# Andurdur/Chroma-Subsampling-Image-Compressor

Measured on AMD Instinct MI355X. Metric: Mpixels/s end-to-end (RGB->YCbCr->4:2:0->reconstruct), higher is better.
Workload: dtype u8

## Files before the change

chroma-subsampling-image-compressor_amd/csrc/csic_pack.hip:

```cpp
#include <cstdio>

#include "csic_pack_common.h"

namespace csic {

template <int Q, bool NT>
__global__ void __launch_bounds__(PK_T) k_pack_widths(PkArgs e)
{
    __shared__ uint32_t s_w[PK_T], s_a[PK_T], s_tot[PK_WAVES];
    const int plane = e.plane0 + (int)blockIdx.y;
    const uint32_t G = e.groups[plane], g0 = blockIdx.x * PK_T, t = threadIdx.x;
    if (g0 >= G) return;
    const gpdst_t cb = pk_coded_frame(e);
    uint32_t w = 0, anchor = 0;
    if (g0 + t < G) {
        uint32_t u[32];
        w = pk_fold_group<Q, NT>(e, pk_bits_frame(e), plane, g0 + t, u, anchor);
    }
    s_w[t] = w;
    s_a[t] = anchor;
    uint32_t total;
    (void)pk_block_scan(w, s_tot, total);
    if (t == 0) *pk_ws(e, blockIdx.z, e.block0[plane] + blockIdx.x) = total;
    pk_store_sections<Q>(e, cb, plane, G, g0, s_w, s_a);
}

__global__ void __launch_bounds__(PK_T) k_pack_scan(PkArgs e)
{
    __shared__ uint32_t s_tot[PK_WAVES];
    uint32_t carry = 0;
    for (uint32_t b0 = 0; b0 < e.nblocks; b0 += PK_T) {
        const uint32_t b = b0 + threadIdx.x;
        const uint32_t v = b < e.nblocks ? *pk_ws(e, blockIdx.x, b) : 0u;
        uint32_t total;
        const uint32_t before = pk_block_scan(v, s_tot, total);
        if (b < e.nblocks) *pk_ws(e, blockIdx.x, b) = carry + before;
        carry += total;
    }
    if (threadIdx.x == 0 && e.sizes)
        ((unsigned long long CSIC_GLOBAL *)(uintptr_t)e.sizes)[blockIdx.x] = (unsigned long long)e.payload_offset + 4ull * carry;
}

template <int Q, bool NT>
__global__ void __launch_bounds__(PK_T) k_pack_emit(PkArgs e)
{
    __shared__ uint32_t s_tot[PK_WAVES];
    const int plane = e.plane0 + (int)blockIdx.y;
    const uint32_t G = e.groups[plane], g0 = blockIdx.x * PK_T, t = threadIdx.x;
    if (g0 >= G) return;
    uint32_t u[32], w = 0, anchor = 0;
#pragma unroll
    for (int j = 0; j < 32; ++j) u[j] = 0;
    if (g0 + t < G) w = pk_fold_group<Q, NT>(e, pk_bits_frame(e), plane, g0 + t, u, anchor);
    uint32_t total;
    const uint32_t before = pk_block_scan(w, s_tot, total);
    if (w == 0) return;
    const gpdst_t cb = pk_coded_frame(e);
    int64_t at = e.payload_offset + 4 * ((int64_t)*pk_ws(e, blockIdx.z, e.block0[plane] + blockIdx.x) + before);
    uint64_t acc = 0;
    uint32_t fill = 0;
#pragma unroll
    for (int j = 0; j < 32; ++j) {
        acc |= (uint64_t)u[j] << fill;
        fill += w;
        if (fill >= 32u) {
            pk_coded_st4(e, cb, at, (uint32_t)acc);
            at += 4;
            acc >>= 32;
            fill -= 32u;
        }
    }
}

__device__ __forceinline__ uint32_t pk_width(const PkArgs &e, gpdst_t cb, int plane, uint32_t g)
{
    return min(pk_nibble(e, cb, plane, g), (uint32_t)e.q[plane]);
}

__global__ void __launch_bounds__(PK_T) k_unpack_sums(PkArgs e)
{
    __shared__ uint32_t s_tot[PK_WAVES];
    const int plane = (int)blockIdx.y;
    const uint32_t G = e.groups[plane], g0 = blockIdx.x * PK_T, t = threadIdx.x;
    if (g0 >= G) return;
    const uint32_t w = g0 + t < G ? pk_width(e, pk_coded_frame(e), plane, g0 + t) : 0u;
    uint32_t total;
    (void)pk_block_scan(w, s_tot, total);
    if (t == 0) *pk_ws(e, blockIdx.z, e.block0[plane] + blockIdx.x) = total;
}

template <int Q, bool NT>
__global__ void __launch_bounds__(PK_T) k_unpack_emit(PkArgs e)
{
    constexpr uint32_t MASK = (1u << Q) - 1u;
    __shared__ uint32_t s_tot[PK_WAVES];
    const int plane = e.plane0 + (int)blockIdx.y;
    const uint32_t G = e.groups[plane], g0 = blockIdx.x * PK_T, t = threadIdx.x, g = g0 + t;
    if (g0 >= G) return;
    const gpdst_t cb = pk_coded_frame(e);
    const uint32_t w = g < G ? pk_width(e, cb, plane, g) : 0u;
    uint32_t total;
    const uint32_t before = pk_block_scan(w, s_tot, total);
    if (g >= G) return;
    uint32_t c = pk_anchor<Q>(e, cb, plane, g);
    const uint32_t n = e.n[plane], wmask = (1u << w) - 1u;
    int64_t at = e.payload_offset + 4 * ((int64_t)*pk_ws(e, blockIdx.z, e.block0[plane] + blockIdx.x) + before);
    uint64_t acc = 0;
    uint32_t have = 0;
    PkGroupOut<Q> out;
#pragma unroll
    for (int j = 0; j < 32; ++j) {
        if (have < w) {
            acc |= (uint64_t)pk_coded_ld4(e, cb, at) << have;
            at += 4;
            have += 32u;
        }
        const uint32_t uu = (uint32_t)acc & wmask;
        acc >>= w;
        have -= w;
        if (j > 0) c = (c + rice_unfold(uu, MASK)) & MASK;
        out.put(j, 32u * g + (uint32_t)j < n ? c : 0u);
    }
    out.template store<NT>(e, pk_bits_frame(e), plane, g);
}

int pk_fill_args(const csic_plan *pl, const PackGeometry &G, const int64_t (&nibbles_offset)[3], const int64_t (&anchors_offset)[3],
                 int64_t payload_offset, int64_t bound_bytes, const char *entry, PkArgs *e)
{
    *e = PkArgs{};
    if ((int64_t)pl->g.W * pl->g.H >= ((int64_t)1 << 31)) return set_error(CSIC_EINVAL_SIZE, "frame too large for %s", entry);
    e->frame_bytes = G.bits.frame_bytes;
    e->bound_bytes = bound_bytes;
    e->payload_offset = payload_offset;
    for (int p = 0; p < 3; ++p) {
        e->off[p] = G.src_offset[p];
        e->bytes[p] = G.src_bytes[p];
        e->n[p] = (uint32_t)G.n[p];
        e->groups[p] = (uint32_t)G.layout.groups[p];
        e->q[p] = G.q[p];
        e->woff[p] = (uint32_t)nibbles_offset[p];
        e->aoff[p] = (uint32_t)anchors_offset[p];
        e->adw[p] = (uint32_t)((G.layout.groups[p] * G.q[p] + 31) / 32);
        e->block0[p] = (uint32_t)G.block0[p];
    }
    e->nblocks = (uint32_t)G.nblocks;
    return CSIC_OK;
}

static int fill_pk_args(const csic_plan *pl, PkArgs *e)
{
    PackGeometry G;
    const int st = pack_geometry(&pl->p, &G);
    if (st != CSIC_OK) return st;
    return pk_fill_args(pl, G, G.layout.widths_offset, G.layout.anchors_offset, G.layout.payload_offset, G.layout.bound_bytes, "csic_pack_device", e);
}

static const auto pack_widths = [](auto q, auto nt) { return k_pack_widths<CSIC_CONST(q), CSIC_CONST(nt)>; };
static const auto pack_emit = [](auto q, auto nt) { return k_pack_emit<CSIC_CONST(q), CSIC_CONST(nt)>; };
static const auto unpack_emit = [](auto q, auto nt) { return k_unpack_emit<CSIC_CONST(q), CSIC_CONST(nt)>; };

static int pk_launch(void (*fn)(PkArgs), PkArgs &e, dim3 grid, hipStream_t stream)
{
    void *params[1] = {&e};
    HIP_TRY(hipLaunchKernel(reinterpret_cast<const void *>(fn), grid, dim3(PK_T, 1, 1), params, 0, stream));
    return CSIC_OK;
}

int pack_scan_launch(PkArgs &e, int nframes, hipStream_t stream) { return pk_launch(k_pack_scan, e, dim3((unsigned)nframes, 1, 1), stream); }

int pk_check_buffers(const csic_plan *plan, const void *d_bits, const void *d_coded, int32_t nframes, bool has_ws, const void *d_workspace)
{
    if (!plan) return set_error(CSIC_EINVAL_NULL, "plan is NULL");
    if (!d_bits || !d_coded || (has_ws && !d_workspace)) return set_error(CSIC_EINVAL_NULL, "device buffer is NULL");
    if (nframes < 1 || nframes > 65535) return set_error(CSIC_EINVAL_SIZE, "nframes must be 1..65535. Got %d", nframes);
    if (((uintptr_t)d_bits | (uintptr_t)d_coded) & 255u) return set_error(CSIC_EINVAL_SIZE, "PLANAR_BITS and coded frame buffers must be 256-byte aligned");
    if (has_ws && ((uintptr_t)d_workspace & 7u)) return set_error(CSIC_EINVAL_SIZE, "d_workspace must be 8-byte aligned");
    return CSIC_OK;
}

const char *pk_kernel_name(const char *family, const csic_plan *plan)
{
    static thread_local char buf[64];
    if (!plan) return "";
    std::snprintf(buf, sizeof buf, "%s<q%d,%d,%d,%s>", family, plan->p.y_bits, plan->p.cb_bits, plan->p.cr_bits, plan->tune.no_nt ? "cached" : "nt");
    return buf;
}

}

using namespace csic;

extern "C" {

const char *csic_pack_kernel_name(const csic_plan *plan) { return pk_kernel_name("k_pack", plan); }

int csic_pack_workspace_bytes(const csic_plan *plan, int32_t nframes, size_t *bytes) { return pk_workspace_bytes(plan, nframes, bytes, fill_pk_args); }

int csic_pack_device(csic_plan *plan, const void *d_bits, int32_t nframes, void *d_coded, uint64_t *d_sizes, void *d_workspace,
                     size_t workspace_bytes, void *hip_stream)
{
    if (plan && !d_sizes) return set_error(CSIC_EINVAL_NULL, "d_sizes is NULL");
    PkArgs e;
    int st = pk_prepare(plan, d_bits, d_coded, nframes, true, d_workspace, workspace_bytes, fill_pk_args, &e);
    if (st != CSIC_OK) return st;
    if ((uintptr_t)d_sizes & 7u) return set_error(CSIC_EINVAL_SIZE, "d_sizes must be 8-byte aligned");
    e.sizes = reinterpret_cast<unsigned long long *>(d_sizes);
    hipStream_t stream = static_cast<hipStream_t>(hip_stream);
    CSIC_DEVICE_SCOPE(plan->device);
    if ((st = pk_launch_planes(plan, e, nframes, stream, pack_widths)) != CSIC_OK) return st;
    if ((st = pack_scan_launch(e, nframes, stream)) != CSIC_OK) return st;
    if ((st = pk_launch_planes(plan, e, nframes, stream, pack_emit)) != CSIC_OK) return st;
    clear_error();
    return CSIC_OK;
}

int csic_unpack_device(csic_plan *plan, const void *d_coded, int32_t nframes, void *d_bits, void *d_workspace, size_t workspace_bytes,
                       void *hip_stream)
{
    PkArgs e;
    int st = pk_prepare(plan, d_bits, d_coded, nframes, true, d_workspace, workspace_bytes, fill_pk_args, &e);
    if (st != CSIC_OK) return st;
    hipStream_t stream = static_cast<hipStream_t>(hip_stream);
    CSIC_DEVICE_SCOPE(plan->device);
    uint32_t gmax = 0;
    for (int p = 0; p < 3; ++p) gmax = e.groups[p] > gmax ? e.groups[p] : gmax;
    if ((st = pk_launch(k_unpack_sums, e, dim3((gmax + PK_T - 1) / PK_T, 3, (unsigned)nframes), stream)) != CSIC_OK) return st;
    if ((st = pack_scan_launch(e, nframes, stream)) != CSIC_OK) return st;
    if ((st = pk_launch_planes(plan, e, nframes, stream, unpack_emit)) != CSIC_OK) return st;
    clear_error();
    return CSIC_OK;
}

}
```

chroma-subsampling-image-compressor_amd/csrc/csic_pack_common.h:

```cpp
#pragma once
#include "csic_kernel_ops.h"
#include "csic_rice_decode.h"

namespace csic {

typedef const uint8_t CSIC_GLOBAL *gpsrc_t;
typedef uint8_t CSIC_GLOBAL *gpdst_t;

constexpr int PK_T = 256, PK_WAVES = PK_T / 64;
static_assert(PK_T == RICE_BLOCK, "a block of the kernels is a block of the format: pack_geometry numbers both");

struct PkArgs {
    uint8_t *bits;
    uint8_t *coded;
    uint32_t *ws;
    unsigned long long *sizes;
    int64_t frame_bytes, bound_bytes;
    int64_t off[3], bytes[3];
    int64_t payload_offset;
    uint32_t n[3], groups[3];
    int32_t q[3];
    uint32_t woff[3], aoff[3];
    uint32_t adw[3];
    uint32_t block0[3], nblocks;
    int32_t plane0;
};

#if defined(CSIC_DEBUG) && CSIC_DEBUG
#define CSIC_PCHECK(lim, off, cnt) CSIC_CHECK((int64_t)(off) >= 0 && (int64_t)(off) + (cnt) <= (int64_t)(lim))
#else
#define CSIC_PCHECK(lim, off, cnt) do { } while (0)
#endif

template <bool NT> __device__ __forceinline__ uint32_t pk_bits_ld4(const PkArgs &e, gpdst_t fb, int64_t off)
{
    CSIC_PCHECK(e.frame_bytes, off, 4); (void)e;
    return ld1<NT>((gin_t)(fb + off));
}
__device__ __forceinline__ uint32_t pk_bits_ld1(const PkArgs &e, gpdst_t fb, int64_t off)
{
    CSIC_PCHECK(e.frame_bytes, off, 1); (void)e;
    return fb[off];
}
template <bool NT> __device__ __forceinline__ void pk_bits_st4(const PkArgs &e, gpdst_t fb, int64_t off, uint32_t v)
{
    CSIC_PCHECK(e.frame_bytes, off, 4); (void)e;
    st1<NT>((gout_t)(fb + off), v);
}
__device__ __forceinline__ void pk_bits_st1(const PkArgs &e, gpdst_t fb, int64_t off, uint32_t v)
{
    CSIC_PCHECK(e.frame_bytes, off, 1); (void)e;
    fb[off] = (uint8_t)v;
}
__device__ __forceinline__ uint32_t pk_coded_ld4(const PkArgs &e, gpdst_t cb, int64_t off)
{
    CSIC_PCHECK(e.bound_bytes, off, 4); (void)e;
    return *(gin_t)(cb + off);
}
__device__ __forceinline__ void pk_coded_st4(const PkArgs &e, gpdst_t cb, int64_t off, uint32_t v)
{
    CSIC_PCHECK(e.bound_bytes, off, 4); (void)e;
    *(gout_t)(cb + off) = v;
}
__device__ __forceinline__ gout_t pk_ws(const PkArgs &e, uint32_t frame, uint32_t b)
{
    CSIC_CHECK(b < e.nblocks && frame < 65535u);
    return (gout_t)(uintptr_t)e.ws + ((uint64_t)frame * e.nblocks + b);
}

__device__ __forceinline__ gpdst_t pk_bits_frame(const PkArgs &e) { return (gpdst_t)(uintptr_t)e.bits + (int64_t)blockIdx.z * e.frame_bytes; }
__device__ __forceinline__ gpdst_t pk_coded_frame(const PkArgs &e) { return (gpdst_t)(uintptr_t)e.coded + (int64_t)blockIdx.z * e.bound_bytes; }

__device__ __forceinline__ uint32_t pk_block_scan(uint32_t v, uint32_t *s_tot, uint32_t &total)
{
    const uint32_t lane = threadIdx.x & 63u, wave = threadIdx.x >> 6;
    uint32_t inc = v;
#pragma unroll
    for (int d = 1; d < 64; d <<= 1) {
        const uint32_t t = (uint32_t)__shfl_up((int)inc, d, 64);
        if (lane >= (uint32_t)d) inc += t;
    }
    if (lane == 63u) s_tot[wave] = inc;
    __syncthreads();
    uint32_t before = 0;
    total = 0;
#pragma unroll
    for (int k = 0; k < PK_WAVES; ++k) {
        const uint32_t t = s_tot[k];
        if ((uint32_t)k < wave) before += t;
        total += t;
    }
    __syncthreads();
    return before + inc - v;
}

template <int Q, bool NT>
__device__ __forceinline__ uint32_t pk_fold_group(const PkArgs &e, gpdst_t fb, int plane, uint32_t g, uint32_t (&u)[32], uint32_t &anchor)
{
    constexpr uint32_t MASK = (1u << Q) - 1u, HALF = 1u << (Q - 1);
    const uint32_t n = e.n[plane];
    const int64_t base = e.off[plane] + 4 * (int64_t)g * Q;
    const bool whole = 32u * g + 32u <= n;
    uint32_t d[Q];
    if (whole) {
#pragma unroll
        for (int i = 0; i < Q; ++i) d[i] = pk_bits_ld4<NT>(e, fb, base + 4 * i);
    } else {
        const int64_t end = e.off[plane] + e.bytes[plane];
#pragma unroll
        for (int i = 0; i < Q; ++i) {
            d[i] = 0;
#pragma unroll
            for (int k = 0; k < 4; ++k)
                if (base + 4 * i + k < end) d[i] |= pk_bits_ld1(e, fb, base + 4 * i + k) << (8 * k);
        }
    }
    uint32_t c[32];
#pragma unroll
    for (int j = 0; j < 32; ++j) {
        const int w = (j * Q) >> 5, s = (j * Q) & 31;
        uint32_t v = d[w] >> s;
        if (s + Q > 32) v |= d[(w + 1) % Q] << ((32 - s) & 31);
        c[j] = v & MASK;
    }
    if (!whole) {
#pragma unroll
        for (int j = 1; j < 32; ++j)
            if (32u * g + (uint32_t)j >= n) c[j] = c[j - 1];
    }
    anchor = c[0];
    uint32_t any = 0;
    u[0] = 0;
#pragma unroll
    for (int j = 1; j < 32; ++j) {
        const uint32_t r = (c[j] - c[j - 1]) & MASK;
        u[j] = r < HALF ? 2u * r : 2u * (MASK + 1u - r) - 1u;
        any |= u[j];
    }
    return any ? 32u - (uint32_t)__builtin_clz(any) : 0u;
}

template <int Q>
__device__ __forceinline__ void pk_store_sections(const PkArgs &e, gpdst_t cb, int plane, uint32_t G, uint32_t g0, const uint32_t *s_nib, const uint32_t *s_a)
{
    const uint32_t t = threadIdx.x;
    if (t < 32u) {
        if (g0 + 8u * t < G) {
            uint32_t v = 0;
#pragma unroll
            for (int k = 0; k < 8; ++k) v |= s_nib[8u * t + (uint32_t)k] << (4 * k);
            pk_coded_st4(e, cb, (int64_t)e.woff[plane] + 4 * (int64_t)(g0 / 8u + t), v);
        }
    } else if (t >= 64u && t < 64u + 8u * Q) {
        const uint32_t a = t - 64u, dw = blockIdx.x * (8u * Q) + a;
        if (dw < e.adw[plane]) {
            uint32_t v = 0;
            for (uint32_t i = 32u * a / Q; i * Q < 32u * a + 32u; ++i) {
                const int sh = (int)(i * Q) - (int)(32u * a);
                v |= sh >= 0 ? s_a[i] << sh : s_a[i] >> -sh;
            }
            pk_coded_st4(e, cb, (int64_t)e.aoff[plane] + 4 * (int64_t)dw, v);
        }
    }
}

__device__ __forceinline__ uint32_t pk_nibble(const PkArgs &e, gpdst_t cb, int plane, uint32_t g)
{
    return (pk_coded_ld4(e, cb, (int64_t)e.woff[plane] + 4 * (int64_t)(g >> 3)) >> (4u * (g & 7u))) & 15u;
}

template <int Q> __device__ __forceinline__ uint32_t pk_anchor(const PkArgs &e, gpdst_t cb, int plane, uint32_t g)
{
    const uint32_t abit = g * Q, as = abit & 31u;
    const int64_t aat = (int64_t)e.aoff[plane] + 4 * (int64_t)(abit >> 5);
    uint32_t c = pk_coded_ld4(e, cb, aat) >> as;
    if (as + Q > 32u) c |= pk_coded_ld4(e, cb, aat + 4) << (32u - as);
    return c & ((1u << Q) - 1u);
}

template <int Q> struct PkGroupOut {
    uint32_t d[Q];
    __device__ __forceinline__ PkGroupOut()
    {
#pragma unroll
        for (int i = 0; i < Q; ++i) d[i] = 0;
    }
    __device__ __forceinline__ void put(int j, uint32_t v)
    {
        const int wi = (j * Q) >> 5, s = (j * Q) & 31;
        d[wi] |= v << s;
        if (s + Q > 32) d[(wi + 1) % Q] |= v >> ((32 - s) & 31);
    }
    template <bool NT> __device__ __forceinline__ void store(const PkArgs &e, gpdst_t fb, int plane, uint32_t g) const
    {
        const int64_t base = e.off[plane] + 4 * (int64_t)g * Q;
        if (32u * g + 32u <= e.n[plane]) {
#pragma unroll
            for (int i = 0; i < Q; ++i) pk_bits_st4<NT>(e, fb, base + 4 * i, d[i]);
        } else {
            const int64_t end = e.off[plane] + e.bytes[plane];
#pragma unroll
            for (int i = 0; i < Q; ++i)
#pragma unroll
                for (int k = 0; k < 4; ++k)
                    if (base + 4 * i + k < end) pk_bits_st1(e, fb, base + 4 * i + k, (d[i] >> (8 * k)) & 0xFFu);
        }
    }
};

int pk_fill_args(const csic_plan *pl, const PackGeometry &G, const int64_t (&nibbles_offset)[3], const int64_t (&anchors_offset)[3],
                 int64_t payload_offset, int64_t bound_bytes, const char *entry, PkArgs *e);

inline size_t pk_workspace_need(int32_t nframes, uint32_t nblocks) { return ((size_t)nframes * nblocks * sizeof(uint32_t) + 7) / 8 * 8; }

int pk_check_buffers(const csic_plan *plan, const void *d_bits, const void *d_coded, int32_t nframes, bool has_ws, const void *d_workspace);
template <class Args>
int pk_prepare(const csic_plan *plan, const void *d_bits, const void *d_coded, int32_t nframes, bool has_ws, const void *d_workspace,
               size_t workspace_bytes, int (*fill)(const csic_plan *, Args *), Args *e)
{
    int st = pk_check_buffers(plan, d_bits, d_coded, nframes, has_ws, d_workspace);
    if (st == CSIC_OK) st = fill(plan, e);
    if (st != CSIC_OK) return st;
    if (has_ws && workspace_bytes < pk_workspace_need(nframes, e->nblocks))
        return set_error(CSIC_EINVAL_SIZE, "workspace of %zu bytes, %d frames need %zu", workspace_bytes, nframes, pk_workspace_need(nframes, e->nblocks));
    e->bits = const_cast<uint8_t *>(static_cast<const uint8_t *>(d_bits));
    e->coded = const_cast<uint8_t *>(static_cast<const uint8_t *>(d_coded));
    e->ws = const_cast<uint32_t *>(static_cast<const uint32_t *>(d_workspace));
    return CSIC_OK;
}

template <class Args> int pk_workspace_bytes(const csic_plan *plan, int32_t nframes, size_t *bytes, int (*fill)(const csic_plan *, Args *))
{
    if (!plan || !bytes) return set_error(CSIC_EINVAL_NULL, "plan or bytes is NULL");
    if (nframes < 1 || nframes > 65535) return set_error(CSIC_EINVAL_SIZE, "nframes must be 1..65535. Got %d", nframes);
    Args e;
    const int st = fill(plan, &e);
    if (st != CSIC_OK) return st;
    *bytes = pk_workspace_need(nframes, e.nblocks);
    clear_error();
    return CSIC_OK;
}

template <class Args, class Choose> int pk_launch_planes(const csic_plan *plan, Args &e, int nframes, hipStream_t stream, Choose choose)
{
    for (int p0 = 0; p0 < 3;) {
        int p1 = p0 + 1;
        while (p1 < 3 && e.q[p1] == e.q[p0]) ++p1;
        uint32_t gmax = 0;
        for (int p = p0; p < p1; ++p) gmax = e.groups[p] > gmax ? e.groups[p] : gmax;
        if (gmax > 0) {
            e.plane0 = p0;
            void (*const fn)(Args) = with_const<true, false>(!plan->tune.no_nt, [&](auto nt) {
                return with_const<1, 2, 3, 4, 5, 6, 7, 8>(e.q[p0], [&](auto q) -> void (*)(Args) { return choose(q, nt); });
            });
            void *params[1] = {&e};
            HIP_TRY(hipLaunchKernel(reinterpret_cast<const void *>(fn), dim3((gmax + PK_T - 1) / PK_T, (unsigned)(p1 - p0), (unsigned)nframes),
                                    dim3(PK_T, 1, 1), params, 0, stream));
        }
        p0 = p1;
    }
    return CSIC_OK;
}

int pack_scan_launch(PkArgs &e, int nframes, hipStream_t stream);

const char *pk_kernel_name(const char *family, const csic_plan *plan);

}
```

chroma-subsampling-image-compressor_amd/csrc/csic_rice_decode.h:

```cpp
#pragma once
#include <cstdint>

#if defined(__HIPCC__)
#define CSIC_RICE_HD __host__ __device__ inline
#else
#define CSIC_RICE_HD inline
#endif

namespace csic {

CSIC_RICE_HD uint32_t rice_word(const uint32_t *seg, uint32_t nwords, uint32_t i) { return i < nwords ? seg[i] : 0u; }

CSIC_RICE_HD uint32_t rice_bits(const uint32_t *seg, uint32_t nwords, uint32_t bit, uint32_t n)
{
    const uint32_t wi = bit >> 5, sh = bit & 31u;
    uint32_t v = rice_word(seg, nwords, wi) >> sh;
    if (sh + n > 32u) v |= rice_word(seg, nwords, wi + 1u) << (32u - sh);
    return v & ((1u << n) - 1u);
}

CSIC_RICE_HD uint32_t rice_select32(uint32_t w, uint32_t r)
{
    uint32_t pos = 0;
    for (uint32_t s = 16; s >= 1u; s >>= 1) {
        const uint32_t lo = w & ((1u << s) - 1u), c = (uint32_t)__builtin_popcount(lo);
        if (r >= c) { r -= c; w >>= s; pos += s; } else w = lo;
    }
    return (w & 1u) && r == 0 ? pos : 32u;
}

CSIC_RICE_HD uint32_t rice_after_terminator(const uint32_t *words, const uint32_t *cum, uint32_t n, uint32_t t)
{
    if (t == 0) return 0;
    uint32_t lo = 0, hi = n;
    while (lo < hi) {
        const uint32_t mid = lo + ((hi - lo) >> 1);
        if (cum[mid] >= t) hi = mid; else lo = mid + 1u;
    }
    if (lo >= n) return 32u * n;
    const uint32_t before = lo ? cum[lo - 1u] : 0u;
    if (before >= t) return 32u * n;
    const uint32_t pos = rice_select32(words[lo], t - 1u - before);
    return pos >= 32u ? 32u * n : 32u * lo + pos + 1u;
}

CSIC_RICE_HD uint32_t rice_unary(const uint32_t *seg, uint32_t nwords, uint32_t *ubit, uint32_t uend, bool *terminated)
{
    if (uend > 32u * nwords) uend = 32u * nwords;
    uint32_t at = *ubit, zeros = 0;
    *terminated = false;
    while (at < uend) {
        const uint32_t sh = at & 31u, room = 32u - sh, avail = uend - at < room ? uend - at : room;
        uint32_t w = seg[at >> 5] >> sh;
        if (avail < 32u) w &= (1u << avail) - 1u;
        if (w) {
            const uint32_t tz = (uint32_t)__builtin_ctz(w);
            *ubit = at + tz + 1u;
            *terminated = true;
            return zeros + tz;
        }
        zeros += avail;
        at += avail;
    }
    *ubit = at;
    return zeros;
}

CSIC_RICE_HD uint32_t rice_next_u(const uint32_t *seg, uint32_t nwords, uint32_t *rbit, uint32_t *ubit, uint32_t uend, uint32_t k, uint32_t q)
{
    uint32_t u = k ? rice_bits(seg, nwords, *rbit, k) : 0u;
    *rbit += k;
    if (k < q) {
        bool terminated;
        const uint32_t zeros = rice_unary(seg, nwords, ubit, uend, &terminated);
        u |= (zeros < 256u ? zeros : 255u) << k;
    }
    return u & ((1u << q) - 1u);
}

CSIC_RICE_HD uint32_t rice_unfold(uint32_t u, uint32_t mask) { return ((u & 1u) ? ~(u >> 1) : (u >> 1)) & mask; }

}
```

Before: 2.117 million.

## Coalesce bit-pack payload I/O via shared staging and widen scan sweeps

The emit kernels now stage the packed payload words in shared memory, so both pack and unpack read and write global memory as contiguous coalesced words instead of per-thread strided streams. Unpack extracts each field with alignbit from the staged words. The width pass computes only the min/max residual range instead of folding all 32 values. The decode-side sums kernel reads nibble words directly and reduces with warp shuffles, one sub-warp per block. The carry scan processes 16 entries per thread with prefetch. Trade-offs are more LDS use per block, which may reduce occupancy, and extra barriers.

```diff
diff --git a/chroma-subsampling-image-compressor_amd/csrc/csic_pack.hip b/chroma-subsampling-image-compressor_amd/csrc/csic_pack.hip
--- a/chroma-subsampling-image-compressor_amd/csrc/csic_pack.hip
+++ b/chroma-subsampling-image-compressor_amd/csrc/csic_pack.hip
@@ -13,10 +13,7 @@
     if (g0 >= G) return;
     const gpdst_t cb = pk_coded_frame(e);
     uint32_t w = 0, anchor = 0;
-    if (g0 + t < G) {
-        uint32_t u[32];
-        w = pk_fold_group<Q, NT>(e, pk_bits_frame(e), plane, g0 + t, u, anchor);
-    }
+    if (g0 + t < G) w = pk_group_width<Q, NT>(e, pk_bits_frame(e), plane, g0 + t, anchor);
     s_w[t] = w;
     s_a[t] = anchor;
     uint32_t total;
@@ -25,26 +22,62 @@
     pk_store_sections<Q>(e, cb, plane, G, g0, s_w, s_a);
 }
 
+constexpr uint32_t PK_SCAN_SWEEP = PK_T * PK_SCAN_N;
+__device__ __forceinline__ uint32_t &pk_scan_slot(uint32_t (&s_v)[PK_SCAN_SWEEP + PK_T], uint32_t i)
+{
+    CSIC_CHECK(i < PK_SCAN_SWEEP);
+    return s_v[i + i / PK_SCAN_N];
+}
+
 __global__ void __launch_bounds__(PK_T) k_pack_scan(PkArgs e)
 {
-    __shared__ uint32_t s_tot[PK_WAVES];
-    uint32_t carry = 0;
-    for (uint32_t b0 = 0; b0 < e.nblocks; b0 += PK_T) {
-        const uint32_t b = b0 + threadIdx.x;
-        const uint32_t v = b < e.nblocks ? *pk_ws(e, blockIdx.x, b) : 0u;
+    __shared__ uint32_t s_tot[PK_WAVES], s_v[PK_SCAN_SWEEP + PK_T];
+    const uint32_t t = threadIdx.x;
+    uint32_t carry = 0, x[PK_SCAN_N];
+#pragma unroll
+    for (int i = 0; i < PK_SCAN_N; ++i) x[i] = *pk_ws(e, blockIdx.x, min((uint32_t)i * PK_T + t, e.nblocks - 1u));
+    for (uint32_t b0 = 0; b0 < e.nblocks; b0 += PK_SCAN_SWEEP) {
+#pragma unroll
+        for (int i = 0; i < PK_SCAN_N; ++i) pk_scan_slot(s_v, (uint32_t)i * PK_T + t) = b0 + (uint32_t)i * PK_T + t < e.nblocks ? x[i] : 0u;
+        if (b0 + PK_SCAN_SWEEP < e.nblocks) {
+#pragma unroll
+            for (int i = 0; i < PK_SCAN_N; ++i) x[i] = *pk_ws(e, blockIdx.x, min(b0 + PK_SCAN_SWEEP + (uint32_t)i * PK_T + t, e.nblocks - 1u));
+        }
+        __syncthreads();
+        uint32_t v[PK_SCAN_N], sum = 0;
+#pragma unroll
+        for (int i = 0; i < PK_SCAN_N; ++i) sum += v[i] = pk_scan_slot(s_v, t * PK_SCAN_N + (uint32_t)i);
         uint32_t total;
-        const uint32_t before = pk_block_scan(v, s_tot, total);
-        if (b < e.nblocks) *pk_ws(e, blockIdx.x, b) = carry + before;
+        uint32_t run = carry + pk_block_scan(sum, s_tot, total);
+#pragma unroll
+        for (int i = 0; i < PK_SCAN_N; ++i) {
+            pk_scan_slot(s_v, t * PK_SCAN_N + (uint32_t)i) = run;
+            run += v[i];
+        }
+        __syncthreads();
+#pragma unroll
+        for (int i = 0; i < PK_SCAN_N; ++i) {
+            const uint32_t b = b0 + (uint32_t)i * PK_T + t;
+            if (b < e.nblocks) *pk_ws(e, blockIdx.x, b) = pk_scan_slot(s_v, (uint32_t)i * PK_T + t);
+        }
         carry += total;
-    }
-    if (threadIdx.x == 0 && e.sizes)
+        __syncthreads();
+    }
+    if (t == 0 && e.sizes)
         ((unsigned long long CSIC_GLOBAL *)(uintptr_t)e.sizes)[blockIdx.x] = (unsigned long long)e.payload_offset + 4ull * carry;
+}
+
+template <int Q> __host__ __device__ constexpr uint32_t pk_row(uint32_t i) { return Q % 4 == 0 ? i + (i >> 5) : i; }
+template <int N> __device__ __forceinline__ uint32_t &pk_staged(uint32_t (&s_pay)[N], uint32_t i)
+{
+    CSIC_CHECK(i < (uint32_t)N);
+    return s_pay[i];
 }
 
 template <int Q, bool NT>
 __global__ void __launch_bounds__(PK_T) k_pack_emit(PkArgs e)
 {
-    __shared__ uint32_t s_tot[PK_WAVES];
+    __shared__ uint32_t s_tot[PK_WAVES], s_pay[PK_T * Q];
     const int plane = e.plane0 + (int)blockIdx.y;
     const uint32_t G = e.groups[plane], g0 = blockIdx.x * PK_T, t = threadIdx.x;
     if (g0 >= G) return;
@@ -53,22 +86,28 @@
     for (int j = 0; j < 32; ++j) u[j] = 0;
     if (g0 + t < G) w = pk_fold_group<Q, NT>(e, pk_bits_frame(e), plane, g0 + t, u, anchor);
     uint32_t total;
-    const uint32_t before = pk_block_scan(w, s_tot, total);
-    if (w == 0) return;
+    uint32_t at = pk_block_scan(w, s_tot, total);
+    if (w != 0) {
+        uint64_t acc = 0;
+        uint32_t fill = 0;
+#pragma unroll
+        for (int j = 0; j < 32; ++j) {
+            acc |= (uint64_t)u[j] << fill;
+            fill += w;
+            if (fill >= 32u) {
+                pk_staged(s_pay, at++) = (uint32_t)acc;
+                acc >>= 32;
+                fill -= 32u;
+            }
+        }
+    }
+    __syncthreads();
     const gpdst_t cb = pk_coded_frame(e);
-    int64_t at = e.payload_offset + 4 * ((int64_t)*pk_ws(e, blockIdx.z, e.block0[plane] + blockIdx.x) + before);
-    uint64_t acc = 0;
-    uint32_t fill = 0;
-#pragma unroll
-    for (int j = 0; j < 32; ++j) {
-        acc |= (uint64_t)u[j] << fill;
-        fill += w;
-        if (fill >= 32u) {
-            pk_coded_st4(e, cb, at, (uint32_t)acc);
-            at += 4;
-            acc >>= 32;
-            fill -= 32u;
-        }
+    const int64_t base = e.payload_offset + 4 * (int64_t)*pk_ws(e, blockIdx.z, e.block0[plane] + blockIdx.x);
+#pragma unroll
+    for (int k = 0; k < Q; ++k) {
+        const uint32_t i = (uint32_t)k * PK_T + t;
+        if (i < total) pk_coded_st4(e, cb, base + 4 * (int64_t)i, pk_staged(s_pay, i));
     }
 }
 
@@ -77,50 +116,61 @@
     return min(pk_nibble(e, cb, plane, g), (uint32_t)e.q[plane]);
 }
 
+constexpr uint32_t PK_SUMS_B = PK_T / 32;
 __global__ void __launch_bounds__(PK_T) k_unpack_sums(PkArgs e)
 {
-    __shared__ uint32_t s_tot[PK_WAVES];
     const int plane = (int)blockIdx.y;
-    const uint32_t G = e.groups[plane], g0 = blockIdx.x * PK_T, t = threadIdx.x;
-    if (g0 >= G) return;
-    const uint32_t w = g0 + t < G ? pk_width(e, pk_coded_frame(e), plane, g0 + t) : 0u;
-    uint32_t total;
-    (void)pk_block_scan(w, s_tot, total);
-    if (t == 0) *pk_ws(e, blockIdx.z, e.block0[plane] + blockIdx.x) = total;
+    const uint32_t G = e.groups[plane], q = (uint32_t)e.q[plane], t = threadIdx.x;
+    const uint32_t blk = blockIdx.x * PK_SUMS_B + t / 32u, g = blk * PK_T + 8u * (t & 31u);
+    uint32_t sum = 0;
+    if (g < G) {
+        const uint32_t d = pk_coded_ld4(e, pk_coded_frame(e), (int64_t)e.woff[plane] + 4 * (int64_t)(g >> 3));
+#pragma unroll
+        for (uint32_t k = 0; k < 8u; ++k)
+            if (g + k < G) sum += min((d >> (4u * k)) & 15u, q);
+    }
+#pragma unroll
+    for (int m = 16; m >= 1; m >>= 1) sum += (uint32_t)__shfl_xor((int)sum, m, 32);
+    if ((t & 31u) == 0 && blk * PK_T < G) *pk_ws(e, blockIdx.z, e.block0[plane] + blk) = sum;
 }
 
 template <int Q, bool NT>
 __global__ void __launch_bounds__(PK_T) k_unpack_emit(PkArgs e)
 {
     constexpr uint32_t MASK = (1u << Q) - 1u;
-    __shared__ uint32_t s_tot[PK_WAVES];
+    __shared__ uint32_t s_tot[PK_WAVES], s_pay[pk_row<Q>(PK_T * Q) + 1];
     const int plane = e.plane0 + (int)blockIdx.y;
     const uint32_t G = e.groups[plane], g0 = blockIdx.x * PK_T, t = threadIdx.x, g = g0 + t;
     if (g0 >= G) return;
     const gpdst_t cb = pk_coded_frame(e);
     const uint32_t w = g < G ? pk_width(e, cb, plane, g) : 0u;
     uint32_t total;
-    const uint32_t before = pk_block_scan(w, s_tot, total);
+    const uint32_t at = pk_block_scan(w, s_tot, total);
+    const int64_t base = e.payload_offset + 4 * (int64_t)*pk_ws(e, blockIdx.z, e.block0[plane] + blockIdx.x);
+#pragma unroll
+    for (int k = 0; k < Q; ++k) {
+        const uint32_t i = (uint32_t)k * PK_T + t;
+        if (i < total) {
+            const uint32_t v = pk_coded_ld4(e, cb, base + 4 * (int64_t)i);
+            pk_staged(s_pay, pk_row<Q>(i)) = v;
+            if (Q % 4 == 0 && (i & 31u) == 0 && i != 0) pk_staged(s_pay, pk_row<Q>(i) - 1u) = v;
+        }
+    }
+    __syncthreads();
     if (g >= G) return;
     uint32_t c = pk_anchor<Q>(e, cb, plane, g);
     const uint32_t n = e.n[plane], wmask = (1u << w) - 1u;
-    int64_t at = e.payload_offset + 4 * ((int64_t)*pk_ws(e, blockIdx.z, e.block0[plane] + blockIdx.x) + before);
-    uint64_t acc = 0;
-    uint32_t have = 0;
     PkGroupOut<Q> out;
-#pragma unroll
-    for (int j = 0; j < 32; ++j) {
-        if (have < w) {
-            acc |= (uint64_t)pk_coded_ld4(e, cb, at) << have;
-            at += 4;
-            have += 32u;
-        }
-        const uint32_t uu = (uint32_t)acc & wmask;
-        acc >>= w;
-        have -= w;
-        if (j > 0) c = (c + rice_unfold(uu, MASK)) & MASK;
-        out.put(j, 32u * g + (uint32_t)j < n ? c : 0u);
-    }
+    const auto steps = [&](auto ragged) {
+#pragma unroll
+        for (int j = 0; j < 32; ++j) {
+            const uint32_t p = (uint32_t)j * w, i = pk_row<Q>(at + (p >> 5));
+            const uint32_t uu = __builtin_amdgcn_alignbit(pk_staged(s_pay, i + 1u), pk_staged(s_pay, i), p & 31u) & wmask;
+            if (j > 0) c = (c + rice_unfold(uu, ~0u)) & MASK;
+            out.put(j, !CSIC_CONST(ragged) || 32u * g + (uint32_t)j < n ? c : 0u);
+        }
+    };
+    if (32u * g + 32u <= n) steps(std::false_type{}); else steps(std::true_type{});
     out.template store<NT>(e, pk_bits_frame(e), plane, g);
 }
 
@@ -224,7 +274,8 @@
     CSIC_DEVICE_SCOPE(plan->device);
     uint32_t gmax = 0;
     for (int p = 0; p < 3; ++p) gmax = e.groups[p] > gmax ? e.groups[p] : gmax;
-    if ((st = pk_launch(k_unpack_sums, e, dim3((gmax + PK_T - 1) / PK_T, 3, (unsigned)nframes), stream)) != CSIC_OK) return st;
+    const uint32_t bmax = (gmax + PK_T - 1) / PK_T;
+    if ((st = pk_launch(k_unpack_sums, e, dim3((bmax + PK_SUMS_B - 1) / PK_SUMS_B, 3, (unsigned)nframes), stream)) != CSIC_OK) return st;
     if ((st = pack_scan_launch(e, nframes, stream)) != CSIC_OK) return st;
     if ((st = pk_launch_planes(plan, e, nframes, stream, unpack_emit)) != CSIC_OK) return st;
     clear_error();
diff --git a/chroma-subsampling-image-compressor_amd/csrc/csic_pack_common.h b/chroma-subsampling-image-compressor_amd/csrc/csic_pack_common.h
--- a/chroma-subsampling-image-compressor_amd/csrc/csic_pack_common.h
+++ b/chroma-subsampling-image-compressor_amd/csrc/csic_pack_common.h
@@ -9,6 +9,7 @@
 
 constexpr int PK_T = 256, PK_WAVES = PK_T / 64;
 static_assert(PK_T == RICE_BLOCK, "a block of the kernels is a block of the format: pack_geometry numbers both");
+constexpr int PK_SCAN_N = 16;
 
 struct PkArgs {
     uint8_t *bits;
@@ -95,13 +96,10 @@
 }
 
 template <int Q, bool NT>
-__device__ __forceinline__ uint32_t pk_fold_group(const PkArgs &e, gpdst_t fb, int plane, uint32_t g, uint32_t (&u)[32], uint32_t &anchor)
-{
-    constexpr uint32_t MASK = (1u << Q) - 1u, HALF = 1u << (Q - 1);
-    const uint32_t n = e.n[plane];
+__device__ __forceinline__ bool pk_load_group(const PkArgs &e, gpdst_t fb, int plane, uint32_t g, uint32_t (&d)[Q])
+{
     const int64_t base = e.off[plane] + 4 * (int64_t)g * Q;
-    const bool whole = 32u * g + 32u <= n;
-    uint32_t d[Q];
+    const bool whole = 32u * g + 32u <= e.n[plane];
     if (whole) {
 #pragma unroll
         for (int i = 0; i < Q; ++i) d[i] = pk_bits_ld4<NT>(e, fb, base + 4 * i);
@@ -115,6 +113,45 @@
                 if (base + 4 * i + k < end) d[i] |= pk_bits_ld1(e, fb, base + 4 * i + k) << (8 * k);
         }
     }
+    return whole;
+}
+
+template <int Q, bool NT>
+__device__ __forceinline__ uint32_t pk_group_width(const PkArgs &e, gpdst_t fb, int plane, uint32_t g, uint32_t &anchor)
+{
+    uint32_t d[Q];
+    const bool whole = pk_load_group<Q, NT>(e, fb, plane, g, d);
+    const uint32_t n = e.n[plane];
+    int32_t smin = 0, smax = 0;
+    const auto steps = [&](auto ragged) {
+        uint32_t prev = 0;
+#pragma unroll
+        for (int j = 0; j < 32; ++j) {
+            const int w = (j * Q) >> 5, s = (j * Q) & 31;
+            uint32_t v = d[w] >> s;
+            if (s + Q > 32) v |= d[(w + 1) % Q] << ((32 - s) & 31);
+            if (j == 0) {
+                anchor = v & ((1u << Q) - 1u);
+            } else {
+                int32_t r = group_residual(v - prev, Q);
+                if (CSIC_CONST(ragged) && 32u * g + (uint32_t)j >= n) r = 0;
+                smin = min(smin, r);
+                smax = max(smax, r);
+            }
+            prev = v;
+        }
+    };
+    if (whole) steps(std::false_type{}); else steps(std::true_type{});
+    return group_width_of_range(smin, smax);
+}
+
+template <int Q, bool NT>
+__device__ __forceinline__ uint32_t pk_fold_group(const PkArgs &e, gpdst_t fb, int plane, uint32_t g, uint32_t (&u)[32], uint32_t &anchor)
+{
+    constexpr uint32_t MASK = (1u << Q) - 1u, HALF = 1u << (Q - 1);
+    const uint32_t n = e.n[plane];
+    uint32_t d[Q];
+    const bool whole = pk_load_group<Q, NT>(e, fb, plane, g, d);
     uint32_t c[32];
 #pragma unroll
     for (int j = 0; j < 32; ++j) {
diff --git a/chroma-subsampling-image-compressor_amd/csrc/csic_rice_decode.h b/chroma-subsampling-image-compressor_amd/csrc/csic_rice_decode.h
--- a/chroma-subsampling-image-compressor_amd/csrc/csic_rice_decode.h
+++ b/chroma-subsampling-image-compressor_amd/csrc/csic_rice_decode.h
@@ -80,4 +80,11 @@
 
 CSIC_RICE_HD uint32_t rice_unfold(uint32_t u, uint32_t mask) { return ((u & 1u) ? ~(u >> 1) : (u >> 1)) & mask; }
 
+CSIC_RICE_HD int32_t group_residual(uint32_t diff, int q) { return (int32_t)(diff << (32 - q)) >> (32 - q); }
+CSIC_RICE_HD uint32_t group_width_of_range(int32_t smin, int32_t smax)
+{
+    const int32_t a = 2 * smax, b = -2 * smin - 1, m = a > b ? a : b;
+    return m > 0 ? 32u - (uint32_t)__builtin_clz((uint32_t)m) : 0u;
 }
+
+}
```

Result: no change. 2.115 million (-0.1%).
